# mightypirate1/DRL-Tetris

Measured on AMD Instinct MI355X. Metric: env-steps/sec at 64k parallel 20x10 boards, higher is better.
Workload: dtype u32

## Files before the change

### drl-tetris_amd/csrc/tetris_engine.h

```cpp
#pragma once
#include "tetris_layout.h"
#include "tetris_tables.h"

#if defined(__clang__)
#define TE_UNROLL _Pragma("unroll")
#else
#define TE_UNROLL _Pragma("GCC unroll 8")
#endif

namespace te {

TE_HD int ctz32(uint32_t v) { return __builtin_ctz(v); }
TE_HD int clz32(uint32_t v) { return __builtin_clz(v); }
#if defined(__HIP_DEVICE_COMPILE__)
TE_HD uint32_t ld_stream(const uint32_t* p) { return __builtin_nontemporal_load(p); }
TE_HD void st_stream(uint32_t* p, uint32_t v) { __builtin_nontemporal_store(v, p); }
#else
TE_HD uint32_t ld_stream(const uint32_t* p) { return *p; }
TE_HD void st_stream(uint32_t* p, uint32_t v) { *p = v; }
#endif

#if defined(TE_PATH_COUNTERS) && !defined(__HIPCC__)
enum PathCounter { PC_KICK = 0, PC_KICK_2ND, PC_KICK_3RD, PC_KICK_FAILED, PC_KICK_DOWN, PC_DROP_EXACT, PC_RT_OFF_SPAWN,
                   PC_GARBAGE_ROW, PC_GARBAGE_LIFT2, PC_DEATH_GARBAGE, PC_DEATH_SPAWN, PC_TIMER_LOCK, PC_KEY_KICK, PC_KEY_KICK_FAILED,
                   PC_UNDO_SIMPLE, PC_UNDO_FULL, PC_UNDO_MISPREDICT, PC_NCOUNTERS };
extern unsigned long long te_path_count[PC_NCOUNTERS];
#define TE_COUNT(i) (te_path_count[i]++)
#else
#define TE_COUNT(i) do {} while (0)
#endif

enum MemMode : int { MEM_STREAM = 0, MEM_AGENT = 1, MEM_AFFINE = 2 };
#if defined(__HIP_DEVICE_COMPILE__)
TE_HD uint32_t ld_agent(const uint32_t* p) { return __hip_atomic_load(p, __ATOMIC_RELAXED, __HIP_MEMORY_SCOPE_AGENT); }
TE_HD void st_agent(uint32_t* p, uint32_t v) { __hip_atomic_store(p, v, __ATOMIC_RELAXED, __HIP_MEMORY_SCOPE_AGENT); }
#else
TE_HD uint32_t ld_agent(const uint32_t* p) { return *p; }
TE_HD void st_agent(uint32_t* p, uint32_t v) { *p = v; }
#endif
#if defined(__HIP_DEVICE_COMPILE__)
TE_HD __amdgpu_buffer_rsrc_t te_rsrc(const void* base) {
    return __builtin_amdgcn_make_buffer_rsrc(const_cast<void*>(base), (short)0, -1, 0x00020000);
}
constexpr int TE_AUX_NT = 2, TE_AUX_SC1 = 16;
TE_HD uint32_t ldw_b(const uint32_t* base, uint32_t o, size_t row_bytes, int mem = MEM_STREAM) {
    const __amdgpu_buffer_rsrc_t r = te_rsrc(base);
    if (mem == MEM_AGENT || mem == MEM_AFFINE) return __builtin_amdgcn_raw_buffer_load_b32(r, (int)o, (int)(uint32_t)row_bytes, TE_AUX_SC1);
    return __builtin_amdgcn_raw_buffer_load_b32(r, (int)o, (int)(uint32_t)row_bytes, TE_AUX_NT);
}
TE_HD void stw_b(uint32_t* base, uint32_t o, size_t row_bytes, uint32_t v, int mem = MEM_STREAM) {
    const __amdgpu_buffer_rsrc_t r = te_rsrc(base);
    if (mem == MEM_AGENT) __builtin_amdgcn_raw_buffer_store_b32(v, r, (int)o, (int)(uint32_t)row_bytes, TE_AUX_SC1);
    else if (mem == MEM_AFFINE) __builtin_amdgcn_raw_buffer_store_b32(v, r, (int)o, (int)(uint32_t)row_bytes, 0);
    else __builtin_amdgcn_raw_buffer_store_b32(v, r, (int)o, (int)(uint32_t)row_bytes, TE_AUX_NT);
}
#else
TE_HD uint32_t ldw_b(const uint32_t* base, uint32_t o, size_t row_bytes, int mem = MEM_STREAM) {
    const uint32_t* p = (const uint32_t*)((const char*)base + row_bytes + o);
    return mem != MEM_STREAM ? ld_agent(p) : ld_stream(p);
}
TE_HD void stw_b(uint32_t* base, uint32_t o, size_t row_bytes, uint32_t v, int mem = MEM_STREAM) {
    uint32_t* p = (uint32_t*)((char*)base + row_bytes + o);
    if (mem != MEM_STREAM) st_agent(p, v); else st_stream(p, v);
}
#endif
TE_HD uint32_t ldw(const uint32_t* base, uint32_t o, size_t word_off, int mem = MEM_STREAM) { return ldw_b(base, o, word_off * 4u, mem); }
TE_HD void stw(uint32_t* base, uint32_t o, size_t word_off, uint32_t v, int mem = MEM_STREAM) { stw_b(base, o, word_off * 4u, v, mem); }
struct RowStride { size_t ws; };
template <int N>
struct RowTable { uint32_t bytes[N]; };
TE_HD size_t row_bytes(const RowStride& r, int w) { return (size_t)w * r.ws * 4u; }
template <int N>
TE_HD size_t row_bytes(const RowTable<N>& r, int w) { return r.bytes[w]; }
#if defined(__HIP_DEVICE_COMPILE__)
TE_HD void add_word(uint32_t* p, uint32_t v) { (void)__hip_atomic_fetch_add(p, v, __ATOMIC_RELAXED, __HIP_MEMORY_SCOPE_AGENT); }
#else
TE_HD void add_word(uint32_t* p, uint32_t v) { *p += v; }
#endif
#if defined(__HIP_DEVICE_COMPILE__)
TE_HD uint32_t mul24(uint32_t a, uint32_t b) { return __umul24(a, b); }
#else
TE_HD uint32_t mul24(uint32_t a, uint32_t b) { return a * b; }
#endif
TE_HD int imin(int a, int b) { return a < b ? a : b; }
TE_HD int imax(int a, int b) { return a > b ? a : b; }
TE_HD uint32_t f2u(float f) { union { float f; uint32_t u; } v; v.f = f; return v.u; }
TE_HD float u2f(uint32_t u) { union { float f; uint32_t u; } v; v.u = u; return v.f; }

constexpr uint16_t SHAPE_ROWS[7][4] = {
    {0x2260, 0x0710, 0x3220, 0x4700}, {0x2230, 0x1700, 0x6220, 0x0740}, {0x2640, 0x0630, 0x1320, 0x6300},
    {0x2310, 0x3600, 0x4620, 0x0360}, {0x2222, 0x0f00, 0x4444, 0x00f0}, {0x0720, 0x2320, 0x2700, 0x2620},
    {0x0660, 0x0660, 0x0660, 0x0660},
};
TE_HD int spawn_rot(int kind) { return (int)((0x0977u >> (2 * (kind & 7))) & 3u); }
TE_HD int shape_value(int kind) { return (int)((0x06127534u >> (4 * (kind & 7))) & 15u); }

// ... 71 lines not shown
    int q_loaded;
    Raw8 pf_raw;
    int pf_ok;
};

struct ResetPrefetch { uint32_t seed16; uint64_t word; int ok; };

template <int P>
struct Game {
    Player pl[P];
    uint32_t seed16;
    int round_over, last_winner;
    uint32_t flags;
    uint32_t episode;
    uint32_t steps;
    uint32_t add_lines, add_sent;
    uint32_t status;
    uint32_t draw0, draw1;
};

template <class ROWS>
TE_HD void load_player_rows(const uint32_t* s, uint32_t o, const ROWS& rows, Player& q, bool tint, bool queue = true, int mem = MEM_STREAM,
                            bool errs = true) {
    for (int c = 0; c < NCOL; c++) q.col[c] = ldw_b(s, o, row_bytes(rows, W_COL0 + c), mem);
    if (tint)
        for (int k = 0; k < 3; k++)
            for (int c = 0; c < NCOL; c++) q.tint[k][c] = ldw_b(s, o, row_bytes(rows, W_TINT0 + 10 * k + c), mem);
    uint32_t w = ldw_b(s, o, row_bytes(rows, W_PIECE), mem);
    q.kind = w & 7; q.rot = (w >> 3) & 3; q.x = (int)((w >> 5) & 15) - 4; q.y = (w >> 9) & 31;
    q.next = (w >> 14) & 7; q.dead = (w >> 17) & 1; q.lock_armed = (w >> 18) & 1; q.reward = (w >> 19) & 255;
    w = ldw_b(s, o, row_bytes(rows, W_MISC), mem);
    q.inc_count = w & 255; q.combo_count = (w >> 8) & 255; q.line_count = (w >> 16) & 255;
    q.qlen = (w >> 24) & 15; q.q_overflow = (w >> 28) & 3;
    if (!queue) { q.inc_count = 0; q.qlen = 0; }
    if (!queue && !errs) q.q_overflow = 0;
    q.time_ms = (int32_t)ldw_b(s, o, row_bytes(rows, W_TIME), mem);
    w = ldw_b(s, o, row_bytes(rows, W_DROPCOMBO), mem);
    q.drop_delay = w & 0xFFFF; q.combo_remaining = w >> 16;
    q.drop_time = (int32_t)ldw_b(s, o, row_bytes(rows, W_DROP_TIME), mem);
    q.speedup_time = (int32_t)ldw_b(s, o, row_bytes(rows, W_SPEEDUP_TIME), mem);
    q.lock_time = (int32_t)ldw_b(s, o, row_bytes(rows, W_LOCK_TIME), mem);
    q.combo_start = (int32_t)ldw_b(s, o, row_bytes(rows, W_COMBO_START), mem);
    q.combo_time = (int32_t)ldw_b(s, o, row_bytes(rows, W_COMBO_TIME), mem);
    q.incoming = queue ? u2f(ldw_b(s, o, row_bytes(rows, W_INCOMING), mem)) : 0.0f;
    q.min_remaining = queue ? (int32_t)ldw_b(s, o, row_bytes(rows, W_MIN_REMAINING), mem) : 1000;
    q.piece_draws = ldw_b(s, o, row_bytes(rows, W_PIECE_DRAWS), mem);
    q.hole_draws = queue ? ldw_b(s, o, row_bytes(rows, W_HOLE_DRAWS), mem) : 0u;
    q.pgroup = ldw_b(s, o, row_bytes(rows, W_PIECE_GROUP), mem);
    w = ldw_b(s, o, row_bytes(rows, W_STATS0), mem); q.lines_sent = w & 0xFFFF; q.lines_cleared = w >> 16;
    w = ldw_b(s, o, row_bytes(rows, W_STATS1), mem); q.lines_blocked = w & 0xFFFF; q.max_combo = w >> 16;
    w = ldw_b(s, o, row_bytes(rows, W_STATS2), mem); q.lines_seen = w & 0xFFFF; q.garbage_cleared = w >> 16;
    q.q_loaded = queue && q.qlen > 0;
    q.pf_ok = 0; q.pf_raw.lo = 0; q.pf_raw.hi = 0;
    if (queue)
        for (int i = 0; i < FIFO_CAP; i++) { q.qcount[i] = 0; q.qdelay[i] = 0; }
    if (q.q_loaded) {
        for (int i = 0; i < FIFO_CAP / 2; i++) {
            uint32_t cw = ldw_b(s, o, row_bytes(rows, W_FIFO_COUNT0 + i), mem);
            q.qcount[2 * i] = (int16_t)(cw & 0xFFFF);
            q.qcount[2 * i + 1] = (int16_t)(cw >> 16);
        }
        for (int i = 0; i < FIFO_CAP; i++) q.qdelay[i] = (int32_t)ldw_b(s, o, row_bytes(rows, W_FIFO_DELAY0 + i), mem);
    }
}

TE_HD void load_player(const uint32_t* s, uint32_t o, size_t ws, Player& q, bool tint, bool queue = true, int mem = MEM_STREAM) {
    load_player_rows(s, o, RowStride{ws}, q, tint, queue, mem);
}

template <int P, class ROWS>
TE_HD void load_game_words_rows(const Ref& gr, const ROWS& rows, Game<P>& g, bool counters = false, int mem = MEM_STREAM) {
    uint32_t meta = ldw_b(gr.s, gr.o, row_bytes(rows, G_META), mem);
    g.seed16 = meta & 0xFFFFu;
    g.round_over = (meta >> 16) & 1;
    g.last_winner = (int)((meta >> 17) & 0xF) - 1;
    g.flags = (meta >> 21) & 7u;
    g.episode = ldw_b(gr.s, gr.o, row_bytes(rows, G_EPISODE), mem);
    g.steps = counters ? ldw_b(gr.s, gr.o, row_bytes(rows, G_STEPS), mem) : 0u;
    g.add_lines = 0; g.add_sent = 0;
    g.status = 0;
}

template <int P>
TE_HD void load_game_words(const Ref& gr, Game<P>& g, bool counters = false, int mem = MEM_STREAM) {
    load_game_words_rows<P>(gr, RowStride{gr.ws}, g, counters, mem);
}

template <int P, class ROWS, class GROWS>
TE_HD void load_game_rows(const Geo& geo_in, size_t slot, const ROWS& rows, const GROWS& grows, Game<P>& g, bool tint = false, bool queue = true,
                          bool counters = false, int mem = MEM_STREAM) {
    Geo geo = geo_in;
    geo.P = P;
    load_game_words_rows<P>(game_ref(geo, slot), grows, g, counters, mem);
    TE_UNROLL
    for (int p = 0; p < P; p++) {
        const Ref r = board_ref(geo, p, slot);
        load_player_rows(r.s, r.o, rows, g.pl[p], tint, queue, mem, !counters);
    }
}
template <int P>
TE_HD void load_game(const Geo& geo_in, size_t slot, Game<P>& g, bool tint = false, bool queue = true, bool counters = false, int mem = MEM_STREAM) {
    load_game_rows<P>(geo_in, slot, RowStride{(size_t)P * geo_in.stride}, RowStride{geo_in.stride}, g, tint, queue, counters, mem);
}

template <class ROWS>
TE_HD void store_player_rows(uint32_t* s, uint32_t o, const ROWS& rows, const Player& q, bool tint, bool queue = true, int mem = MEM_STREAM) {
    for (int c = 0; c < NCOL; c++) stw_b(s, o, row_bytes(rows, W_COL0 + c), q.col[c], mem);
    if (tint)
        for (int k = 0; k < 3; k++)
            for (int c = 0; c < NCOL; c++) stw_b(s, o, row_bytes(rows, W_TINT0 + 10 * k + c), q.tint[k][c], mem);
    stw_b(s, o, row_bytes(rows, W_PIECE), (uint32_t)q.kind | ((uint32_t)q.rot << 3) | ((uint32_t)(q.x + 4) << 5) | ((uint32_t)q.y << 9) |
                              ((uint32_t)q.next << 14) | ((uint32_t)q.dead << 17) | ((uint32_t)q.lock_armed << 18) |
                              ((uint32_t)(q.reward & 255) << 19), mem);
    stw_b(s, o, row_bytes(rows, W_MISC), (uint32_t)(q.inc_count & 255) | ((uint32_t)(q.combo_count & 255) << 8) |
                             ((uint32_t)(q.line_count & 255) << 16) | ((uint32_t)q.qlen << 24) | ((uint32_t)q.q_overflow << 28), mem);
    stw_b(s, o, row_bytes(rows, W_TIME), (uint32_t)q.time_ms, mem);
    stw_b(s, o, row_bytes(rows, W_DROPCOMBO), ((uint32_t)q.drop_delay & 0xFFFF) | (q.combo_remaining << 16), mem);
    stw_b(s, o, row_bytes(rows, W_DROP_TIME), (uint32_t)q.drop_time, mem);
    stw_b(s, o, row_bytes(rows, W_SPEEDUP_TIME), (uint32_t)q.speedup_time, mem);
    stw_b(s, o, row_bytes(rows, W_LOCK_TIME), (uint32_t)q.lock_time, mem);
    stw_b(s, o, row_bytes(rows, W_COMBO_START), (uint32_t)q.combo_start, mem);
    stw_b(s, o, row_bytes(rows, W_COMBO_TIME), (uint32_t)q.combo_time, mem);
    if (queue) stw_b(s, o, row_bytes(rows, W_INCOMING), f2u(q.incoming), mem);
    stw_b(s, o, row_bytes(rows, W_MIN_REMAINING), (uint32_t)q.min_remaining, mem);
    stw_b(s, o, row_bytes(rows, W_PIECE_DRAWS), q.piece_draws, mem);
    if (queue) stw_b(s, o, row_bytes(rows, W_HOLE_DRAWS), q.hole_draws, mem);
    stw_b(s, o, row_bytes(rows, W_PIECE_GROUP), q.pgroup, mem);
    stw_b(s, o, row_bytes(rows, W_STATS0), (q.lines_sent & 0xFFFF) | (q.lines_cleared << 16), mem);
    stw_b(s, o, row_bytes(rows, W_STATS1), (q.lines_blocked & 0xFFFF) | (q.max_combo << 16), mem);
    stw_b(s, o, row_bytes(rows, W_STATS2), (q.lines_seen & 0xFFFF) | (q.garbage_cleared << 16), mem);
    if (queue && (q.q_loaded || q.qlen > 0)) {
        for (int i = 0; i < FIFO_CAP / 2; i++)
            stw_b(s, o, row_bytes(rows, W_FIFO_COUNT0 + i), ((uint32_t)q.qcount[2 * i] & 0xFFFF) | ((uint32_t)q.qcount[2 * i + 1] << 16), mem);
        for (int i = 0; i < FIFO_CAP; i++) stw_b(s, o, row_bytes(rows, W_FIFO_DELAY0 + i), (uint32_t)q.qdelay[i], mem);
    }
}

TE_HD void store_player(uint32_t* s, uint32_t o, size_t ws, const Player& q, bool tint, bool queue = true, int mem = MEM_STREAM) {
    store_player_rows(s, o, RowStride{ws}, q, tint, queue, mem);
}

template <int P, class ROWS>
TE_HD void store_game_words_rows(const Ref& gr, const ROWS& rows, const Game<P>& g, bool counters = false, int mem = MEM_STREAM) {
    stw_b(gr.s, gr.o, row_bytes(rows, G_META), g.seed16 | ((uint32_t)g.round_over << 16) | ((uint32_t)(g.last_winner + 1) << 17) | (g.flags << 21), mem);
    stw_b(gr.s, gr.o, row_bytes(rows, G_EPISODE), g.episode, mem);
    if (counters) stw_b(gr.s, gr.o, row_bytes(rows, G_STEPS), g.steps, mem);
    if (g.add_lines) add_word((uint32_t*)((char*)gr.s + row_bytes(rows, G_LINES) + gr.o), g.add_lines);
    if (g.add_sent) add_word((uint32_t*)((char*)gr.s + row_bytes(rows, G_SENT) + gr.o), g.add_sent);
}

template <int P>
TE_HD void store_game_words(const Ref& gr, const Game<P>& g, bool counters = false, int mem = MEM_STREAM) {
    store_game_words_rows<P>(gr, RowStride{gr.ws}, g, counters, mem);
}

template <int P, class ROWS, class GROWS>
TE_HD void store_game_rows(const Geo& geo_in, size_t slot, const ROWS& rows, const GROWS& grows, const Game<P>& g, bool tint = false, bool queue = true,
                           bool counters = false, int mem = MEM_STREAM) {
    Geo geo = geo_in;
    geo.P = P;
    store_game_words_rows<P>(game_ref(geo, slot), grows, g, counters, mem);
    TE_UNROLL
    for (int p = 0; p < P; p++) {
        const Ref r = board_ref(geo, p, slot);
        store_player_rows(r.s, r.o, rows, g.pl[p], tint, queue, mem);
    }
}
template <int P>
TE_HD void store_game(const Geo& geo_in, size_t slot, const Game<P>& g, bool tint = false, bool queue = true, bool counters = false, int mem = MEM_STREAM) {
    store_game_rows<P>(geo_in, slot, RowStride{(size_t)P * geo_in.stride}, RowStride{geo_in.stride}, g, tint, queue, counters, mem);
}


TE_HD uint32_t shape_of(const Ctx& cx, int kind, int rot) { return cx.shapes[(kind << 2) | rot]; }

TE_HD uint64_t band_window(const Ctx& cx, const Player& q, int y) {
    uint32_t lo = 0xFFu, hi = 0xFFFF0000u;
    for (int c = 0; c < 6; c++) lo |= ((uint32_t)((int32_t)(q.col[c] | cx.floor_bits) >> y) & 0xFu) << (4 * c + 8);
    for (int c = 6; c < NCOL; c++) hi |= ((uint32_t)((int32_t)(q.col[c] | cx.floor_bits) >> y) & 0xFu) << (4 * (c - 6));
    return ((uint64_t)hi << 32) | lo;
}

TE_HD bool fits_band(uint64_t band, uint32_t shape, int x) {
    unsigned xs = (unsigned)(x + 2);
// ... 318 lines not shown
    if (q.lock_armed && q.time_ms > q.lock_time && !soft_drop(cx, q)) {
        TE_COUNT(PC_TIMER_LOCK);
        lock_piece(cx, q);
        sent = settle(cx, q, seed16, status);
        finished = true;
    }
    if (!finished) {
        if (cx.queue) {
            int whole = 0;
            while (q.incoming >= 1.0f) { whole++; q.incoming = q.incoming - 1.f; }
            if (whole) q_add(q, whole, q.time_ms, status);
        }
        sent = combo_expire(cx, q, q.time_ms);
        if (sent) {
            if (cx.queue) sent = q_block(q, sent, q.time_ms, false);
            q.lines_sent = (q.lines_sent + (uint32_t)sent) & 0xFFFFu;
        }
        if (cx.queue && q_release(q, q.time_ms))
            if (push_garbage(cx, q, seed16, status)) sent = -1;
    }
    return sent;
}

TE_HD void restart_player(const Ctx& cx, Player& q, uint32_t seed16, uint32_t& status, const ResetPrefetch* pf = nullptr) {
    for (int c = 0; c < NCOL; c++) q.col[c] = 0;
    if (cx.tint)
        for (int k = 0; k < 3; k++)
            for (int c = 0; c < NCOL; c++) q.tint[k][c] = 0;
    q.qlen = 0; q.q_overflow = 0; q.lines_blocked = 0; q.min_remaining = 1000;
    if (cx.queue)
        for (int i = 0; i < FIFO_CAP; i++) { q.qcount[i] = 0; q.qdelay[i] = 0; }
    q.combo_start = 0; q.combo_time = 0; q.max_combo = 0; q.combo_count = 0; q.line_count = 0;
    q.lines_sent = 0; q.lines_cleared = 0; q.garbage_cleared = 0;
    q.speedup_time = 0; q.drop_delay = 1000; q.drop_time = 0; q.lock_time = 0; q.lock_armed = 0;
    q.time_ms = 0; q.incoming = 0.0f; q.lines_seen = 0; q.dead = 0;
    (void)status;
    const uint64_t word = (pf && pf->ok && pf->seed16 == seed16) ? pf->word : cx.start[seed16];
    const uint32_t j = (uint32_t)word & 0xFFu, b0 = ((uint32_t)word >> 8) & 0xFFu, b1 = ((uint32_t)word >> 16) & 0xFFu;
    q.pgroup = (uint32_t)(word >> 32);
    q.kind = (int)(b0 & 7u);
    q.next = (int)(b1 & 7u);
    q.pf_ok = 0;
    q.rot = spawn_rot(q.kind);
    q.x = (NCOL - 4) / 2; q.y = 0;
    q.piece_draws = j + 2; q.hole_draws = 0;
}

template <int P>
TE_HD void reset_game(const Ctx& cx, Game<P>& g, uint32_t seed16, const ResetPrefetch* pf = nullptr) {
    g.round_over = 0;
    int winner = -1, alive = 0;
    TE_UNROLL
    for (int p = 0; p < P; p++)
        if (!g.pl[p].dead) { alive++; winner = p; }
    g.last_winner = winner;
    if (P == 1) g.last_winner = 0;
    if (alive > 1) g.last_winner = -1;
    g.seed16 = seed16 & 0xFFFFu;
    TE_UNROLL
    for (int p = 0; p < P; p++) restart_player(cx, g.pl[p], g.seed16, g.status, pf);
}

TE_HD void prefetch_reset(const Ctx& cx, uint32_t next_seed16, ResetPrefetch& pf) {
    pf.seed16 = next_seed16 & 0xFFFFu;
    pf.word = cx.start[pf.seed16];
    pf.ok = 1;
}

template <int P>
TE_HD void init_game(const Ctx& cx, Game<P>& g, uint32_t seed16) {
    TE_UNROLL
    for (int p = 0; p < P; p++) {
        Player& q = g.pl[p];
        q.reward = 0; q.inc_count = 0; q.combo_remaining = 0; q.dead = 0; q.next = 0; q.kind = 7; q.rot = 0;
        q.q_loaded = 1;
    }
    g.episode = 0; g.steps = 0; g.add_lines = 0; g.add_sent = 0; g.status = 0; g.flags = 0;
    reset_game(cx, g, seed16);
    g.last_winner = -1;
}


TE_HD bool rotate_shape_band(const Ctx& cx, Player& q, int nr, uint32_t shape, uint64_t& b0, uint64_t& b1, bool& b1_ok) {
// ... 530 lines not shown

TE_HD int split_finish(Game<1>& g, int lines_in, bool opp_dead, bool opp_err = false) {
    Player& q = g.pl[0];
    if (g.round_over) return 1;
    if (lines_in > 0) q.incoming = q.incoming + (float)lines_in / 1.0f;
    g.flags = (g.flags & ~SPLIT_OPP_DEAD) | (opp_dead ? SPLIT_OPP_DEAD : 0u);
    int alive = (q.dead ? 0 : 1) + (opp_dead ? 0 : 1);
    if (alive < 2 || q.q_overflow || opp_err) { g.round_over = 1; return 1; }
    return 0;
}

TE_HD void reset_split(const Ctx& cx, Game<1>& g, uint32_t seed16) {
    const int side = (int)(g.flags & SPLIT_SIDE);
    const bool me_alive = !g.pl[0].dead, opp_alive = !(g.flags & SPLIT_OPP_DEAD);
    int winner = -1;
    if (me_alive && !opp_alive) winner = side;
    if (opp_alive && !me_alive) winner = 1 - side;
    reset_game<1>(cx, g, seed16);
    g.last_winner = winner;
    g.flags &= ~SPLIT_OPP_DEAD;
}

TE_HD uint32_t episode_seed(uint32_t game, uint32_t episode) { return (12345u + mul24(7919u, game & 0xFFFFu) + mul24(104729u & 0xFFFFu, episode & 0xFFFFu)) & 0xFFFFu; }

TE_HD void philox4x32_10(uint32_t k0, uint32_t c0, uint32_t c1, uint32_t c2, uint32_t out[4]) {
    uint32_t k1 = 0u, c3 = 0u;
    TE_UNROLL
    for (int r = 0; r < 10; r++) {
        uint64_t p0 = (uint64_t)0xD2511F53u * c0;
        uint64_t p1 = (uint64_t)0xCD9E8D57u * c2;
        uint32_t n0 = (uint32_t)(p1 >> 32) ^ c1 ^ k0;
        uint32_t n1 = (uint32_t)p1;
        uint32_t n2 = (uint32_t)(p0 >> 32) ^ c3 ^ k1;
        uint32_t n3 = (uint32_t)p0;
        c0 = n0; c1 = n1; c2 = n2; c3 = n3;
        k0 += 0x9E3779B9u; k1 += 0xBB67AE85u;
    }
    out[0] = c0; out[1] = c1; out[2] = c2; out[3] = c3;
}

}
```

### drl-tetris_amd/csrc/tetris_hip.hip

```cpp
#include <hip/hip_runtime.h>
#include <hip/hip_ext.h>

#include <math.h>
#include <stdio.h>
#include <stdlib.h>
#include <string.h>

#include <algorithm>
#include <atomic>
#include <mutex>
#include <thread>
#include <new>
#include <chrono>
#include <string>
#include <vector>

#include "tetris_kernels.h"

using namespace te;


#include "tetris_game_kernel.h"

constexpr int CHAIN_LANES = 64;
constexpr int CHAIN_STREAMS = 3;
template <int P, bool AFFINE, bool FUSED>
__device__ __forceinline__ void chain_body(const KArgs& a) {
    __shared__ __attribute__((aligned(16))) uint32_t s_shapes[SHAPE_WORDS];
    const int lane = threadIdx.x;
    if (a.steps < 0) { chain_census(a, lane == 0); return; }
    constexpr int CMEM = AFFINE ? MEM_AFFINE : MEM_AGENT;
    int wave = blockIdx.x;
    uint32_t xcc = 0;
    const auto report_xcc = [&]() { if (AFFINE && blockIdx.x == 0 && lane == 0) st_flag(a.status + F_XCC0 + (a.xcd_slot & 3u), 0x100u | xcc); };
    if (AFFINE) {
        asm volatile("s_getreg_b32 %0, hwreg(HW_REG_XCC_ID)" : "=s"(xcc));
        xcc &= 0xFu;
        if (xcc != ((a.xcd_base + blockIdx.x) & 7u)) {
            if (lane == 0) st_flag(a.status + F_PLACE, 1u);
            report_xcc();
            return;
        }
        wave = (int)((blockIdx.x & ~7u) | xcc);
        if (wave * CHAIN_LANES >= a.n) { report_xcc(); return; }
    }
    const int i = wave * CHAIN_LANES + lane;
    const bool active = lane < CHAIN_LANES && i < a.n;
    LaneCounters cnt = {0, 0, 0, 0};
    const uint32_t shape_word = d_shape_table.s[lane];
    Game<P> g;
    if (active) policy_draw(a, (uint32_t)i, a.first_step, g.draw0, g.draw1);
    const uint32_t d0 = g.draw0, d1 = g.draw1;
    int stride = a.n_stride;
    asm volatile("" : "+s"(stride));
    RowTable<NWORDS> rows = {};
    RowTable<NGWORDS> grows = {};
    if (!FUSED) {
        TE_UNROLL
        for (int w = 0; w < NWORDS; w++)
            if (P > 1 || (w < NWORDS_HOT && w != W_INCOMING && w != W_HOLE_DRAWS)) {
                uint32_t bytes = (uint32_t)(w * P) * (uint32_t)stride * 4u;
                asm volatile("" : "+s"(bytes));
                rows.bytes[w] = bytes;
            }
        TE_UNROLL
        for (int w = 0; w < NGWORDS; w++) {
            uint32_t bytes = (uint32_t)w * (uint32_t)stride * 4u;
            asm volatile("" : "+s"(bytes));
            grows.bytes[w] = bytes;
        }
    }
    const uint32_t seen = chain_poll(a, (uint32_t)wave);
    if (seen == a.epoch - 1u) {
        Geo geo = geo_of(a);
        geo.stride = (size_t)stride;
        if (active) {
            if (FUSED) load_game<P>(geo, (size_t)i, g, false, P > 1, true, CMEM);
            else load_game_rows<P>(geo, (size_t)i, rows, grows, g, false, P > 1, true, CMEM);
            g.draw0 = d0; g.draw1 = d1;
        }
        s_shapes[lane] = shape_word;
        __builtin_amdgcn_wave_barrier();
        if (FUSED) {
            if (active) game_run<P, M_ROLLOUT, false, CMEM>(a, i, s_shapes, g, cnt);
        } else if (active) {
            const Ctx cx = make_ctx(a, s_shapes, false, P > 1);
            rollout_step<P>(cx, a, (size_t)i, a.first_step, g, cnt);
            store_game_rows<P>(geo, (size_t)i, rows, grows, g, false, P > 1, true, CMEM);
            report_status(a, g.status);
        }
        asm volatile("s_waitcnt vmcnt(0)" ::: "memory");
        if (lane == 0) {
            if (AFFINE) st_xcd(a.chain + (size_t)wave * CHAIN_STRIDE, a.epoch);
            else st_agent(a.chain + (size_t)wave * CHAIN_STRIDE, a.epoch);
        }
    } else if (!(seen & CHAIN_ABANDONED)) {
        chain_give_up(a, (uint32_t)wave, lane == 0);
    }
    report_xcc();
}
template <int P>
__global__ __launch_bounds__(64) void k_chain(KArgs a) { chain_body<P, false, false>(a); }
template <int P>
__global__ __launch_bounds__(64) void k_chain_affine(KArgs a) { chain_body<P, true, false>(a); }
template <int P>
__global__ __launch_bounds__(64) void k_chain_fused(KArgs a) { chain_body<P, false, true>(a); }
template <int P>
__global__ __launch_bounds__(64) void k_chain_fused_affine(KArgs a) { chain_body<P, true, true>(a); }
template __global__ void k_chain_affine<1>(KArgs);
template __global__ void k_chain_fused_affine<1>(KArgs);
extern "C" __global__ void tetris_k_xcc_probe(uint32_t* out) {
    if (threadIdx.x == 0) {
        uint32_t xcc;
        asm volatile("s_getreg_b32 %0, hwreg(HW_REG_XCC_ID)" : "=s"(xcc));
        out[blockIdx.x] = xcc & 0xFu;
    }
}
// ... 2845 lines not shown
```

### drl-tetris_amd/csrc/tetris_kernels.h

```cpp
#pragma once
#include "../../include/tetris_hip.h"
#include "tetris_engine.h"

namespace te {

struct KArgs {
    uint32_t* state;
    uint32_t* gstate;
    uint32_t* status;
    const uint8_t* table;
    const uint64_t* start;
    const double* combo_pow;
    uint32_t n_draws, margin;
    int H;
    int n_games;
    int n_stride;
    int n_players;
    int nw;
    int n;
    const int32_t* idx;
    const uint8_t* keys;
    const uint8_t* lens;
    int max_keys;
    const uint8_t* rot;
// ... 58 lines not shown
constexpr uint32_t CHAIN_ABANDONED = 0x80000000u;
constexpr uint32_t CHAIN_EPOCH_MAX = 0x7FFF0000u;
constexpr int CHAIN_STRIDE = 32;
constexpr int CHAIN_SLEEP = 1;
constexpr uint32_t CHAIN_SPIN_LIMIT = 1u << 22;

#if defined(__HIP_DEVICE_COMPILE__)
typedef __attribute__((address_space(1))) uint32_t te_gu32;
TE_HD void or_agent(uint32_t* p, uint32_t v) { (void)__hip_atomic_fetch_or(p, v, __ATOMIC_RELAXED, __HIP_MEMORY_SCOPE_AGENT); }
TE_HD void st_flag(uint32_t* p, uint32_t v) { __hip_atomic_store((te_gu32*)p, v, __ATOMIC_RELAXED, __HIP_MEMORY_SCOPE_SYSTEM); }
TE_HD uint32_t ld_flag(const uint32_t* p) { return __hip_atomic_load((const te_gu32*)p, __ATOMIC_RELAXED, __HIP_MEMORY_SCOPE_SYSTEM); }
TE_HD void st_xcd(uint32_t* p, uint32_t v) { __hip_atomic_store((te_gu32*)p, v, __ATOMIC_RELAXED, __HIP_MEMORY_SCOPE_WAVEFRONT); }
#else
TE_HD void or_agent(uint32_t* p, uint32_t v) { *p |= v; }
TE_HD void st_flag(uint32_t* p, uint32_t v) { *(volatile uint32_t*)p = v; }
TE_HD uint32_t ld_flag(const uint32_t* p) { return *(const volatile uint32_t*)p; }
TE_HD void st_xcd(uint32_t* p, uint32_t v) { *p = v; }
#endif

TE_HD uint32_t chain_poll(const KArgs& a, uint32_t wave) {
    const uint32_t want = a.epoch - 1u;
    const uint32_t* word = a.chain + (size_t)wave * CHAIN_STRIDE;
    uint32_t v = (uint32_t)wave_uniform(ld_agent(word));
    for (uint32_t polls = 1; v != want && !(v & CHAIN_ABANDONED) && polls < a.chain_spin_limit; polls++) {
        if ((polls & 255u) == 0 && wave_uniform(ld_flag(a.status + F_PLACE)) != 0) break;
#if defined(__HIP_DEVICE_COMPILE__)
        __builtin_amdgcn_s_sleep(CHAIN_SLEEP);
#endif
        v = (uint32_t)wave_uniform(ld_agent(word));
    }
    return v;
}
TE_HD void chain_give_up(const KArgs& a, uint32_t wave, bool marker) {
    if (!marker) return;
    or_agent(a.chain + (size_t)wave * CHAIN_STRIDE, CHAIN_ABANDONED);
    st_flag(a.status + F_CHAIN, 1u);
#if defined(__HIP_DEVICE_COMPILE__)
    asm volatile("s_waitcnt vmcnt(0)" ::: "memory");
#endif
}
TE_HD bool chain_wait(const KArgs& a, uint32_t wave, bool marker) {
    const uint32_t seen = chain_poll(a, wave);
    if (seen == a.epoch - 1u) return true;
    if (!(seen & CHAIN_ABANDONED)) chain_give_up(a, wave, marker);
    return false;
}

TE_HD void chain_census(const KArgs& a, bool marker) {
// ... 49 lines not shown
template <int P>
TE_HD void make_rt(const Ctx& cx, Game<P>& g, int player, int r, int t) {
    if (g.round_over) return;
    TE_UNROLL
    for (int p = 0; p < P; p++)
        if (p == player && !g.pl[p].dead) play_rt(cx, g.pl[p], r, t);
}

TE_HD void policy_draw(const KArgs& a, uint32_t slot, unsigned long long step, uint32_t& w0, uint32_t& w1) {
    uint32_t w[4];
    philox4x32_10(a.policy_seed, a.game_offset + slot, (uint32_t)step, (uint32_t)(step >> 32), w);
    w0 = w[0]; w1 = w[1];
}

template <int P, int MODE, bool TINT = false, int MEM = MEM_STREAM>
TE_HD void game_load(const KArgs& a, int i, Game<P>& g) {
    const size_t slot = a.idx ? (size_t)a.idx[i] : (size_t)i;
    if (MODE != M_INIT && MODE != M_SPLIT_INIT)
        load_game<P>(geo_of(a), slot, g, TINT, P > 1 || MODE == M_SPLIT_RESET, MODE == M_ROLLOUT, MEM);
    if (MODE == M_ROLLOUT) policy_draw(a, (uint32_t)slot, a.first_step, g.draw0, g.draw1);
    if (MODE == M_STEP_RT || MODE == M_STEP_RT_AUTO) { g.draw0 = a.rot[i]; g.draw1 = (uint32_t)a.trans[i] | ((a.player ? (uint32_t)a.player[i] : 0u) << 8); }
}

template <int P>
TE_HD void rollout_step(const Ctx& cx, const KArgs& a, size_t slot, unsigned long long step, Game<P>& g, LaneCounters& cnt) {
    TE_UNROLL
    for (int p = 0; p < P; p++) prefetch_next(cx, g.pl[p], g.seed16, g.status);
    ResetPrefetch rpf;
    prefetch_reset(cx, episode_seed(a.game_offset + (uint32_t)slot, g.episode + 1), rpf);
    int r = (int)(g.draw0 & 3u), t = (int)(g.draw1 % 10u);
    int player = P > 1 ? (int)(step % (unsigned long long)P) : 0;
    uint32_t sent_before = 0;
    TE_UNROLL
    for (int p = 0; p < P; p++) sent_before += g.pl[p].lines_sent;
    make_rt<P>(cx, g, player, r, t);
    int done = finish_game<P>(cx, g, a.ms);
    cnt.steps++;
    g.steps++;
    uint32_t sent_after = 0;
    TE_UNROLL
    for (int p = 0; p < P; p++) {
        sent_after += g.pl[p].lines_sent;
        if (!g.pl[p].dead) { cnt.lines += (unsigned)g.pl[p].reward; g.add_lines += (unsigned)g.pl[p].reward; }
    }
    cnt.sent += (sent_after - sent_before) & 0xFFFFu;
    g.add_sent += (sent_after - sent_before) & 0xFFFFu;
    if (done) {
        cnt.episodes++;
        g.episode++;
        reset_game<P>(cx, g, episode_seed(a.game_offset + (uint32_t)slot, g.episode), &rpf);
    }
}

template <int P, int MODE, bool TINT = false, int MEM = MEM_STREAM>
TE_HD void game_run(const KArgs& a, int i, const uint32_t* shapes, Game<P>& g, LaneCounters& cnt) {
    const size_t slot = a.idx ? (size_t)a.idx[i] : (size_t)i;
    Ctx cx = make_ctx(a, shapes, TINT, P > 1 || MODE == M_SPLIT_INIT || MODE == M_SPLIT_RESET);
    if (MODE == M_INIT) init_game<P>(cx, g, (uint32_t)(a.seeds ? (uint16_t)a.seeds[i] : 0));
    if (MODE == M_SPLIT_INIT) {
        init_game<P>(cx, g, (uint32_t)(a.seeds ? (uint16_t)a.seeds[i] : 0));
        g.flags = SPLIT_ON | (a.steps ? SPLIT_SIDE : 0u);
    } else if (MODE == M_SPLIT_RESET) {
        if (P == 1) reset_split(cx, *reinterpret_cast<Game<1>*>(&g), (uint32_t)(a.seeds ? (uint16_t)a.seeds[i] : 0));
    } else if (MODE == M_RESET) {
        reset_game<P>(cx, g, (uint32_t)(a.seeds ? (uint16_t)a.seeds[i] : 0));
    } else if (MODE == M_RESET_SCHED) {
        g.episode++;
        reset_game<P>(cx, g, episode_seed(a.game_offset + (uint32_t)slot, g.episode));
    } else if (MODE == M_MAKE) {
        make_keys<P>(cx, a, i, g);
    } else if (MODE == M_FINISH) {
        TE_UNROLL
        for (int p = 0; p < P; p++) prefetch_next(cx, g.pl[p], g.seed16, g.status);
// ... 442 lines not shown
```

Before: 22.43 billion.

## Hoist buffer descriptors, precompute episode seeds, and defer counter atomics past chain signal

Builds the buffer resource descriptors for the state arrays once per kernel and keeps them in scalar registers, so per-word loads and stores no longer rebuild the descriptor. It also precomputes the game-dependent part of the episode seed and reuses the prefetched reset word unconditionally. Counter atomics and status reporting are moved after the chain epoch signal so they no longer delay the next wave. The chain poll loop is rewritten with a single bounded countdown. The changes cut scalar and vector overhead in a small, latency-bound step, at the cost of more pinned registers and inline asm.

```diff
diff --git a/drl-tetris_amd/csrc/tetris_engine.h b/drl-tetris_amd/csrc/tetris_engine.h
--- a/drl-tetris_amd/csrc/tetris_engine.h
+++ b/drl-tetris_amd/csrc/tetris_engine.h
@@ -39,22 +39,25 @@
 TE_HD void st_agent(uint32_t* p, uint32_t v) { *p = v; }
 #endif
 #if defined(__HIP_DEVICE_COMPILE__)
-TE_HD __amdgpu_buffer_rsrc_t te_rsrc(const void* base) {
+typedef __amdgpu_buffer_rsrc_t te_rsrc_t;
+TE_HD te_rsrc_t te_rsrc(const void* base) {
     return __builtin_amdgcn_make_buffer_rsrc(const_cast<void*>(base), (short)0, -1, 0x00020000);
 }
 constexpr int TE_AUX_NT = 2, TE_AUX_SC1 = 16;
-TE_HD uint32_t ldw_b(const uint32_t* base, uint32_t o, size_t row_bytes, int mem = MEM_STREAM) {
-    const __amdgpu_buffer_rsrc_t r = te_rsrc(base);
+TE_HD uint32_t ldw_rsrc(te_rsrc_t r, uint32_t o, size_t row_bytes, int mem = MEM_STREAM) {
     if (mem == MEM_AGENT || mem == MEM_AFFINE) return __builtin_amdgcn_raw_buffer_load_b32(r, (int)o, (int)(uint32_t)row_bytes, TE_AUX_SC1);
     return __builtin_amdgcn_raw_buffer_load_b32(r, (int)o, (int)(uint32_t)row_bytes, TE_AUX_NT);
 }
-TE_HD void stw_b(uint32_t* base, uint32_t o, size_t row_bytes, uint32_t v, int mem = MEM_STREAM) {
-    const __amdgpu_buffer_rsrc_t r = te_rsrc(base);
+TE_HD void stw_rsrc(te_rsrc_t r, uint32_t o, size_t row_bytes, uint32_t v, int mem = MEM_STREAM) {
     if (mem == MEM_AGENT) __builtin_amdgcn_raw_buffer_store_b32(v, r, (int)o, (int)(uint32_t)row_bytes, TE_AUX_SC1);
     else if (mem == MEM_AFFINE) __builtin_amdgcn_raw_buffer_store_b32(v, r, (int)o, (int)(uint32_t)row_bytes, 0);
     else __builtin_amdgcn_raw_buffer_store_b32(v, r, (int)o, (int)(uint32_t)row_bytes, TE_AUX_NT);
 }
+TE_HD uint32_t ldw_b(const uint32_t* base, uint32_t o, size_t row_bytes, int mem = MEM_STREAM) { return ldw_rsrc(te_rsrc(base), o, row_bytes, mem); }
+TE_HD void stw_b(uint32_t* base, uint32_t o, size_t row_bytes, uint32_t v, int mem = MEM_STREAM) { stw_rsrc(te_rsrc(base), o, row_bytes, v, mem); }
 #else
+struct te_rsrc_t {};
+TE_HD te_rsrc_t te_rsrc(const void*) { return te_rsrc_t{}; }
 TE_HD uint32_t ldw_b(const uint32_t* base, uint32_t o, size_t row_bytes, int mem = MEM_STREAM) {
     const uint32_t* p = (const uint32_t*)((const char*)base + row_bytes + o);
     return mem != MEM_STREAM ? ld_agent(p) : ld_stream(p);
@@ -72,6 +75,20 @@
 TE_HD size_t row_bytes(const RowStride& r, int w) { return (size_t)w * r.ws * 4u; }
 template <int N>
 TE_HD size_t row_bytes(const RowTable<N>& r, int w) { return r.bytes[w]; }
+template <int N>
+struct RowTableR { uint32_t bytes[N]; te_rsrc_t r; };
+template <int N>
+TE_HD size_t row_bytes(const RowTableR<N>& r, int w) { return r.bytes[w]; }
+template <class ROWS>
+TE_HD uint32_t ldw_r(const ROWS& rows, const uint32_t* base, uint32_t o, int w, int mem) { return ldw_b(base, o, row_bytes(rows, w), mem); }
+template <class ROWS>
+TE_HD void stw_r(const ROWS& rows, uint32_t* base, uint32_t o, int w, uint32_t v, int mem) { stw_b(base, o, row_bytes(rows, w), v, mem); }
+#if defined(__HIP_DEVICE_COMPILE__)
+template <int N>
+TE_HD uint32_t ldw_r(const RowTableR<N>& rows, const uint32_t*, uint32_t o, int w, int mem) { return ldw_rsrc(rows.r, o, rows.bytes[w], mem); }
+template <int N>
+TE_HD void stw_r(const RowTableR<N>& rows, uint32_t*, uint32_t o, int w, uint32_t v, int mem) { stw_rsrc(rows.r, o, rows.bytes[w], v, mem); }
+#endif
 #if defined(__HIP_DEVICE_COMPILE__)
 TE_HD void add_word(uint32_t* p, uint32_t v) { (void)__hip_atomic_fetch_add(p, v, __ATOMIC_RELAXED, __HIP_MEMORY_SCOPE_AGENT); }
 #else
@@ -189,45 +206,45 @@
 template <class ROWS>
 TE_HD void load_player_rows(const uint32_t* s, uint32_t o, const ROWS& rows, Player& q, bool tint, bool queue = true, int mem = MEM_STREAM,
                             bool errs = true) {
-    for (int c = 0; c < NCOL; c++) q.col[c] = ldw_b(s, o, row_bytes(rows, W_COL0 + c), mem);
+    for (int c = 0; c < NCOL; c++) q.col[c] = ldw_r(rows, s, o, W_COL0 + c, mem);
     if (tint)
         for (int k = 0; k < 3; k++)
-            for (int c = 0; c < NCOL; c++) q.tint[k][c] = ldw_b(s, o, row_bytes(rows, W_TINT0 + 10 * k + c), mem);
-    uint32_t w = ldw_b(s, o, row_bytes(rows, W_PIECE), mem);
+            for (int c = 0; c < NCOL; c++) q.tint[k][c] = ldw_r(rows, s, o, W_TINT0 + 10 * k + c, mem);
+    uint32_t w = ldw_r(rows, s, o, W_PIECE, mem);
     q.kind = w & 7; q.rot = (w >> 3) & 3; q.x = (int)((w >> 5) & 15) - 4; q.y = (w >> 9) & 31;
     q.next = (w >> 14) & 7; q.dead = (w >> 17) & 1; q.lock_armed = (w >> 18) & 1; q.reward = (w >> 19) & 255;
-    w = ldw_b(s, o, row_bytes(rows, W_MISC), mem);
+    w = ldw_r(rows, s, o, W_MISC, mem);
     q.inc_count = w & 255; q.combo_count = (w >> 8) & 255; q.line_count = (w >> 16) & 255;
     q.qlen = (w >> 24) & 15; q.q_overflow = (w >> 28) & 3;
     if (!queue) { q.inc_count = 0; q.qlen = 0; }
     if (!queue && !errs) q.q_overflow = 0;
-    q.time_ms = (int32_t)ldw_b(s, o, row_bytes(rows, W_TIME), mem);
-    w = ldw_b(s, o, row_bytes(rows, W_DROPCOMBO), mem);
+    q.time_ms = (int32_t)ldw_r(rows, s, o, W_TIME, mem);
+    w = ldw_r(rows, s, o, W_DROPCOMBO, mem);
     q.drop_delay = w & 0xFFFF; q.combo_remaining = w >> 16;
-    q.drop_time = (int32_t)ldw_b(s, o, row_bytes(rows, W_DROP_TIME), mem);
-    q.speedup_time = (int32_t)ldw_b(s, o, row_bytes(rows, W_SPEEDUP_TIME), mem);
-    q.lock_time = (int32_t)ldw_b(s, o, row_bytes(rows, W_LOCK_TIME), mem);
-    q.combo_start = (int32_t)ldw_b(s, o, row_bytes(rows, W_COMBO_START), mem);
-    q.combo_time = (int32_t)ldw_b(s, o, row_bytes(rows, W_COMBO_TIME), mem);
-    q.incoming = queue ? u2f(ldw_b(s, o, row_bytes(rows, W_INCOMING), mem)) : 0.0f;
-    q.min_remaining = queue ? (int32_t)ldw_b(s, o, row_bytes(rows, W_MIN_REMAINING), mem) : 1000;
-    q.piece_draws = ldw_b(s, o, row_bytes(rows, W_PIECE_DRAWS), mem);
-    q.hole_draws = queue ? ldw_b(s, o, row_bytes(rows, W_HOLE_DRAWS), mem) : 0u;
-    q.pgroup = ldw_b(s, o, row_bytes(rows, W_PIECE_GROUP), mem);
-    w = ldw_b(s, o, row_bytes(rows, W_STATS0), mem); q.lines_sent = w & 0xFFFF; q.lines_cleared = w >> 16;
-    w = ldw_b(s, o, row_bytes(rows, W_STATS1), mem); q.lines_blocked = w & 0xFFFF; q.max_combo = w >> 16;
-    w = ldw_b(s, o, row_bytes(rows, W_STATS2), mem); q.lines_seen = w & 0xFFFF; q.garbage_cleared = w >> 16;
+    q.drop_time = (int32_t)ldw_r(rows, s, o, W_DROP_TIME, mem);
+    q.speedup_time = (int32_t)ldw_r(rows, s, o, W_SPEEDUP_TIME, mem);
+    q.lock_time = (int32_t)ldw_r(rows, s, o, W_LOCK_TIME, mem);
+    q.combo_start = (int32_t)ldw_r(rows, s, o, W_COMBO_START, mem);
+    q.combo_time = (int32_t)ldw_r(rows, s, o, W_COMBO_TIME, mem);
+    q.incoming = queue ? u2f(ldw_r(rows, s, o, W_INCOMING, mem)) : 0.0f;
+    q.min_remaining = queue ? (int32_t)ldw_r(rows, s, o, W_MIN_REMAINING, mem) : 1000;
+    q.piece_draws = ldw_r(rows, s, o, W_PIECE_DRAWS, mem);
+    q.hole_draws = queue ? ldw_r(rows, s, o, W_HOLE_DRAWS, mem) : 0u;
+    q.pgroup = ldw_r(rows, s, o, W_PIECE_GROUP, mem);
+    w = ldw_r(rows, s, o, W_STATS0, mem); q.lines_sent = w & 0xFFFF; q.lines_cleared = w >> 16;
+    w = ldw_r(rows, s, o, W_STATS1, mem); q.lines_blocked = w & 0xFFFF; q.max_combo = w >> 16;
+    w = ldw_r(rows, s, o, W_STATS2, mem); q.lines_seen = w & 0xFFFF; q.garbage_cleared = w >> 16;
     q.q_loaded = queue && q.qlen > 0;
     q.pf_ok = 0; q.pf_raw.lo = 0; q.pf_raw.hi = 0;
     if (queue)
         for (int i = 0; i < FIFO_CAP; i++) { q.qcount[i] = 0; q.qdelay[i] = 0; }
     if (q.q_loaded) {
         for (int i = 0; i < FIFO_CAP / 2; i++) {
-            uint32_t cw = ldw_b(s, o, row_bytes(rows, W_FIFO_COUNT0 + i), mem);
+            uint32_t cw = ldw_r(rows, s, o, W_FIFO_COUNT0 + i, mem);
             q.qcount[2 * i] = (int16_t)(cw & 0xFFFF);
             q.qcount[2 * i + 1] = (int16_t)(cw >> 16);
         }
-        for (int i = 0; i < FIFO_CAP; i++) q.qdelay[i] = (int32_t)ldw_b(s, o, row_bytes(rows, W_FIFO_DELAY0 + i), mem);
+        for (int i = 0; i < FIFO_CAP; i++) q.qdelay[i] = (int32_t)ldw_r(rows, s, o, W_FIFO_DELAY0 + i, mem);
     }
 }
 
@@ -237,13 +254,13 @@
 
 template <int P, class ROWS>
 TE_HD void load_game_words_rows(const Ref& gr, const ROWS& rows, Game<P>& g, bool counters = false, int mem = MEM_STREAM) {
-    uint32_t meta = ldw_b(gr.s, gr.o, row_bytes(rows, G_META), mem);
+    uint32_t meta = ldw_r(rows, gr.s, gr.o, G_META, mem);
     g.seed16 = meta & 0xFFFFu;
     g.round_over = (meta >> 16) & 1;
     g.last_winner = (int)((meta >> 17) & 0xF) - 1;
     g.flags = (meta >> 21) & 7u;
-    g.episode = ldw_b(gr.s, gr.o, row_bytes(rows, G_EPISODE), mem);
-    g.steps = counters ? ldw_b(gr.s, gr.o, row_bytes(rows, G_STEPS), mem) : 0u;
+    g.episode = ldw_r(rows, gr.s, gr.o, G_EPISODE, mem);
+    g.steps = counters ? ldw_r(rows, gr.s, gr.o, G_STEPS, mem) : 0u;
     g.add_lines = 0; g.add_sent = 0;
     g.status = 0;
 }
@@ -272,34 +289,34 @@
 
 template <class ROWS>
 TE_HD void store_player_rows(uint32_t* s, uint32_t o, const ROWS& rows, const Player& q, bool tint, bool queue = true, int mem = MEM_STREAM) {
-    for (int c = 0; c < NCOL; c++) stw_b(s, o, row_bytes(rows, W_COL0 + c), q.col[c], mem);
+    for (int c = 0; c < NCOL; c++) stw_r(rows, s, o, W_COL0 + c, q.col[c], mem);
     if (tint)
         for (int k = 0; k < 3; k++)
-            for (int c = 0; c < NCOL; c++) stw_b(s, o, row_bytes(rows, W_TINT0 + 10 * k + c), q.tint[k][c], mem);
-    stw_b(s, o, row_bytes(rows, W_PIECE), (uint32_t)q.kind | ((uint32_t)q.rot << 3) | ((uint32_t)(q.x + 4) << 5) | ((uint32_t)q.y << 9) |
+            for (int c = 0; c < NCOL; c++) stw_r(rows, s, o, W_TINT0 + 10 * k + c, q.tint[k][c], mem);
+    stw_r(rows, s, o, W_PIECE, (uint32_t)q.kind | ((uint32_t)q.rot << 3) | ((uint32_t)(q.x + 4) << 5) | ((uint32_t)q.y << 9) |
                               ((uint32_t)q.next << 14) | ((uint32_t)q.dead << 17) | ((uint32_t)q.lock_armed << 18) |
                               ((uint32_t)(q.reward & 255) << 19), mem);
-    stw_b(s, o, row_bytes(rows, W_MISC), (uint32_t)(q.inc_count & 255) | ((uint32_t)(q.combo_count & 255) << 8) |
+    stw_r(rows, s, o, W_MISC, (uint32_t)(q.inc_count & 255) | ((uint32_t)(q.combo_count & 255) << 8) |
                              ((uint32_t)(q.line_count & 255) << 16) | ((uint32_t)q.qlen << 24) | ((uint32_t)q.q_overflow << 28), mem);
-    stw_b(s, o, row_bytes(rows, W_TIME), (uint32_t)q.time_ms, mem);
-    stw_b(s, o, row_bytes(rows, W_DROPCOMBO), ((uint32_t)q.drop_delay & 0xFFFF) | (q.combo_remaining << 16), mem);
-    stw_b(s, o, row_bytes(rows, W_DROP_TIME), (uint32_t)q.drop_time, mem);
-    stw_b(s, o, row_bytes(rows, W_SPEEDUP_TIME), (uint32_t)q.speedup_time, mem);
-    stw_b(s, o, row_bytes(rows, W_LOCK_TIME), (uint32_t)q.lock_time, mem);
-    stw_b(s, o, row_bytes(rows, W_COMBO_START), (uint32_t)q.combo_start, mem);
-    stw_b(s, o, row_bytes(rows, W_COMBO_TIME), (uint32_t)q.combo_time, mem);
-    if (queue) stw_b(s, o, row_bytes(rows, W_INCOMING), f2u(q.incoming), mem);
-    stw_b(s, o, row_bytes(rows, W_MIN_REMAINING), (uint32_t)q.min_remaining, mem);
-    stw_b(s, o, row_bytes(rows, W_PIECE_DRAWS), q.piece_draws, mem);
-    if (queue) stw_b(s, o, row_bytes(rows, W_HOLE_DRAWS), q.hole_draws, mem);
-    stw_b(s, o, row_bytes(rows, W_PIECE_GROUP), q.pgroup, mem);
-    stw_b(s, o, row_bytes(rows, W_STATS0), (q.lines_sent & 0xFFFF) | (q.lines_cleared << 16), mem);
-    stw_b(s, o, row_bytes(rows, W_STATS1), (q.lines_blocked & 0xFFFF) | (q.max_combo << 16), mem);
-    stw_b(s, o, row_bytes(rows, W_STATS2), (q.lines_seen & 0xFFFF) | (q.garbage_cleared << 16), mem);
+    stw_r(rows, s, o, W_TIME, (uint32_t)q.time_ms, mem);
+    stw_r(rows, s, o, W_DROPCOMBO, ((uint32_t)q.drop_delay & 0xFFFF) | (q.combo_remaining << 16), mem);
+    stw_r(rows, s, o, W_DROP_TIME, (uint32_t)q.drop_time, mem);
+    stw_r(rows, s, o, W_SPEEDUP_TIME, (uint32_t)q.speedup_time, mem);
+    stw_r(rows, s, o, W_LOCK_TIME, (uint32_t)q.lock_time, mem);
+    stw_r(rows, s, o, W_COMBO_START, (uint32_t)q.combo_start, mem);
+    stw_r(rows, s, o, W_COMBO_TIME, (uint32_t)q.combo_time, mem);
+    if (queue) stw_r(rows, s, o, W_INCOMING, f2u(q.incoming), mem);
+    stw_r(rows, s, o, W_MIN_REMAINING, (uint32_t)q.min_remaining, mem);
+    stw_r(rows, s, o, W_PIECE_DRAWS, q.piece_draws, mem);
+    if (queue) stw_r(rows, s, o, W_HOLE_DRAWS, q.hole_draws, mem);
+    stw_r(rows, s, o, W_PIECE_GROUP, q.pgroup, mem);
+    stw_r(rows, s, o, W_STATS0, (q.lines_sent & 0xFFFF) | (q.lines_cleared << 16), mem);
+    stw_r(rows, s, o, W_STATS1, (q.lines_blocked & 0xFFFF) | (q.max_combo << 16), mem);
+    stw_r(rows, s, o, W_STATS2, (q.lines_seen & 0xFFFF) | (q.garbage_cleared << 16), mem);
     if (queue && (q.q_loaded || q.qlen > 0)) {
         for (int i = 0; i < FIFO_CAP / 2; i++)
-            stw_b(s, o, row_bytes(rows, W_FIFO_COUNT0 + i), ((uint32_t)q.qcount[2 * i] & 0xFFFF) | ((uint32_t)q.qcount[2 * i + 1] << 16), mem);
-        for (int i = 0; i < FIFO_CAP; i++) stw_b(s, o, row_bytes(rows, W_FIFO_DELAY0 + i), (uint32_t)q.qdelay[i], mem);
+            stw_r(rows, s, o, W_FIFO_COUNT0 + i, ((uint32_t)q.qcount[2 * i] & 0xFFFF) | ((uint32_t)q.qcount[2 * i + 1] << 16), mem);
+        for (int i = 0; i < FIFO_CAP; i++) stw_r(rows, s, o, W_FIFO_DELAY0 + i, (uint32_t)q.qdelay[i], mem);
     }
 }
 
@@ -307,13 +324,18 @@
     store_player_rows(s, o, RowStride{ws}, q, tint, queue, mem);
 }
 
+template <class ROWS>
+TE_HD void add_game_counters(const Ref& gr, const ROWS& rows, uint32_t add_lines, uint32_t add_sent) {
+    if (add_lines) add_word((uint32_t*)((char*)gr.s + row_bytes(rows, G_LINES) + gr.o), add_lines);
+    if (add_sent) add_word((uint32_t*)((char*)gr.s + row_bytes(rows, G_SENT) + gr.o), add_sent);
+}
+
 template <int P, class ROWS>
-TE_HD void store_game_words_rows(const Ref& gr, const ROWS& rows, const Game<P>& g, bool counters = false, int mem = MEM_STREAM) {
-    stw_b(gr.s, gr.o, row_bytes(rows, G_META), g.seed16 | ((uint32_t)g.round_over << 16) | ((uint32_t)(g.last_winner + 1) << 17) | (g.flags << 21), mem);
-    stw_b(gr.s, gr.o, row_bytes(rows, G_EPISODE), g.episode, mem);
-    if (counters) stw_b(gr.s, gr.o, row_bytes(rows, G_STEPS), g.steps, mem);
-    if (g.add_lines) add_word((uint32_t*)((char*)gr.s + row_bytes(rows, G_LINES) + gr.o), g.add_lines);
-    if (g.add_sent) add_word((uint32_t*)((char*)gr.s + row_bytes(rows, G_SENT) + gr.o), g.add_sent);
+TE_HD void store_game_words_rows(const Ref& gr, const ROWS& rows, const Game<P>& g, bool counters = false, int mem = MEM_STREAM, bool adds = true) {
+    stw_r(rows, gr.s, gr.o, G_META, g.seed16 | ((uint32_t)g.round_over << 16) | ((uint32_t)(g.last_winner + 1) << 17) | (g.flags << 21), mem);
+    stw_r(rows, gr.s, gr.o, G_EPISODE, g.episode, mem);
+    if (counters) stw_r(rows, gr.s, gr.o, G_STEPS, g.steps, mem);
+    if (adds) add_game_counters(gr, rows, g.add_lines, g.add_sent);
 }
 
 template <int P>
@@ -323,10 +345,10 @@
 
 template <int P, class ROWS, class GROWS>
 TE_HD void store_game_rows(const Geo& geo_in, size_t slot, const ROWS& rows, const GROWS& grows, const Game<P>& g, bool tint = false, bool queue = true,
-                           bool counters = false, int mem = MEM_STREAM) {
+                           bool counters = false, int mem = MEM_STREAM, bool adds = true) {
     Geo geo = geo_in;
     geo.P = P;
-    store_game_words_rows<P>(game_ref(geo, slot), grows, g, counters, mem);
+    store_game_words_rows<P>(game_ref(geo, slot), grows, g, counters, mem, adds);
     TE_UNROLL
     for (int p = 0; p < P; p++) {
         const Ref r = board_ref(geo, p, slot);
@@ -691,7 +713,7 @@
     return sent;
 }
 
-TE_HD void restart_player(const Ctx& cx, Player& q, uint32_t seed16, uint32_t& status, const ResetPrefetch* pf = nullptr) {
+TE_HD void restart_player(const Ctx& cx, Player& q, uint32_t seed16, uint32_t& status, const ResetPrefetch* pf = nullptr, bool pf_sure = false) {
     for (int c = 0; c < NCOL; c++) q.col[c] = 0;
     if (cx.tint)
         for (int k = 0; k < 3; k++)
@@ -704,7 +726,7 @@
     q.speedup_time = 0; q.drop_delay = 1000; q.drop_time = 0; q.lock_time = 0; q.lock_armed = 0;
     q.time_ms = 0; q.incoming = 0.0f; q.lines_seen = 0; q.dead = 0;
     (void)status;
-    const uint64_t word = (pf && pf->ok && pf->seed16 == seed16) ? pf->word : cx.start[seed16];
+    const uint64_t word = (pf && (pf_sure || (pf->ok && pf->seed16 == seed16))) ? pf->word : cx.start[seed16];
     const uint32_t j = (uint32_t)word & 0xFFu, b0 = ((uint32_t)word >> 8) & 0xFFu, b1 = ((uint32_t)word >> 16) & 0xFFu;
     q.pgroup = (uint32_t)(word >> 32);
     q.kind = (int)(b0 & 7u);
@@ -716,7 +738,7 @@
 }
 
 template <int P>
-TE_HD void reset_game(const Ctx& cx, Game<P>& g, uint32_t seed16, const ResetPrefetch* pf = nullptr) {
+TE_HD void reset_game(const Ctx& cx, Game<P>& g, uint32_t seed16, const ResetPrefetch* pf = nullptr, bool pf_sure = false) {
     g.round_over = 0;
     int winner = -1, alive = 0;
     TE_UNROLL
@@ -727,7 +749,7 @@
     if (alive > 1) g.last_winner = -1;
     g.seed16 = seed16 & 0xFFFFu;
     TE_UNROLL
-    for (int p = 0; p < P; p++) restart_player(cx, g.pl[p], g.seed16, g.status, pf);
+    for (int p = 0; p < P; p++) restart_player(cx, g.pl[p], g.seed16, g.status, pf, pf_sure);
 }
 
 TE_HD void prefetch_reset(const Ctx& cx, uint32_t next_seed16, ResetPrefetch& pf) {
@@ -1304,6 +1326,17 @@
 }
 
 TE_HD uint32_t episode_seed(uint32_t game, uint32_t episode) { return (12345u + mul24(7919u, game & 0xFFFFu) + mul24(104729u & 0xFFFFu, episode & 0xFFFFu)) & 0xFFFFu; }
+TE_HD uint32_t episode_seed_game(uint32_t game) { return 12345u + mul24(7919u, game & 0xFFFFu); }
+TE_HD uint32_t episode_seed_of(uint32_t game_half, uint32_t episode) {
+#if defined(__HIP_DEVICE_COMPILE__)
+    uint32_t e;
+    asm("v_mul_u32_u24 %0, 0x9919, %1" : "=v"(e) : "v"(episode & 0xFFFFu));
+    static_assert((104729u & 0xFFFFu) == 0x9919u, "episode_seed");
+    return (game_half + e) & 0xFFFFu;
+#else
+    return (game_half + mul24(104729u & 0xFFFFu, episode & 0xFFFFu)) & 0xFFFFu;
+#endif
+}
 
 TE_HD void philox4x32_10(uint32_t k0, uint32_t c0, uint32_t c1, uint32_t c2, uint32_t out[4]) {
     uint32_t k1 = 0u, c3 = 0u;
diff --git a/drl-tetris_amd/csrc/tetris_hip.hip b/drl-tetris_amd/csrc/tetris_hip.hip
--- a/drl-tetris_amd/csrc/tetris_hip.hip
+++ b/drl-tetris_amd/csrc/tetris_hip.hip
@@ -24,6 +24,12 @@
 
 constexpr int CHAIN_LANES = 64;
 constexpr int CHAIN_STREAMS = 3;
+template <class T>
+__device__ __forceinline__ const T* pin_global(const T* p) {
+    unsigned long long u = (unsigned long long)p;
+    asm volatile("" : "+s"(u));
+    return (const T*)(const __attribute__((address_space(1))) T*)u;
+}
 template <int P, bool AFFINE, bool FUSED>
 __device__ __forceinline__ void chain_body(const KArgs& a) {
     __shared__ __attribute__((aligned(16))) uint32_t s_shapes[SHAPE_WORDS];
@@ -53,9 +59,15 @@
     const uint32_t d0 = g.draw0, d1 = g.draw1;
     int stride = a.n_stride;
     asm volatile("" : "+s"(stride));
-    RowTable<NWORDS> rows = {};
-    RowTable<NGWORDS> grows = {};
+    static_assert(FUSED || P == 1, "one board per game: its rows start at KArgs::state");
+    RowTableR<NWORDS> rows = {};
+    RowTableR<NGWORDS> grows = {};
     if (!FUSED) {
+        rows.r = te_rsrc(a.state);
+        grows.r = te_rsrc(a.gstate);
+#if defined(__HIP_DEVICE_COMPILE__)
+        asm volatile("" : "+s"(rows.r), "+s"(grows.r));
+#endif
         TE_UNROLL
         for (int w = 0; w < NWORDS; w++)
             if (P > 1 || (w < NWORDS_HOT && w != W_INCOMING && w != W_HOLE_DRAWS)) {
@@ -70,6 +82,15 @@
             grows.bytes[w] = bytes;
         }
     }
+    StepAhead ahead = {0, a.ms};
+    Ctx cx = make_ctx(a, s_shapes, false, P > 1);
+    if (!FUSED) {
+        ahead.seed_game = episode_seed_game(a.game_offset + (uint32_t)i);
+        asm volatile("" : "+v"(ahead.seed_game));
+        asm volatile("" : "+s"(ahead.ms));
+        asm volatile("" : "+s"(cx.floor_bits));
+        cx.table = pin_global(cx.table); cx.start = pin_global(cx.start); cx.combo_pow = pin_global(cx.combo_pow);
+    }
     const uint32_t seen = chain_poll(a, (uint32_t)wave);
     if (seen == a.epoch - 1u) {
         Geo geo = geo_of(a);
@@ -84,15 +105,20 @@
         if (FUSED) {
             if (active) game_run<P, M_ROLLOUT, false, CMEM>(a, i, s_shapes, g, cnt);
         } else if (active) {
-            const Ctx cx = make_ctx(a, s_shapes, false, P > 1);
-            rollout_step<P>(cx, a, (size_t)i, a.first_step, g, cnt);
-            store_game_rows<P>(geo, (size_t)i, rows, grows, g, false, P > 1, true, CMEM);
-            report_status(a, g.status);
+            rollout_step<P>(cx, a, (size_t)i, a.first_step, g, cnt, &ahead);
+            store_game_rows<P>(geo, (size_t)i, rows, grows, g, false, P > 1, true, CMEM, false);
         }
         asm volatile("s_waitcnt vmcnt(0)" ::: "memory");
         if (lane == 0) {
             if (AFFINE) st_xcd(a.chain + (size_t)wave * CHAIN_STRIDE, a.epoch);
             else st_agent(a.chain + (size_t)wave * CHAIN_STRIDE, a.epoch);
+        }
+        if (!FUSED && active) {
+            add_game_counters(game_ref(geo, (size_t)i), grows, g.add_lines, g.add_sent);
+            if (g.status) {
+                report_status(a, g.status);
+                asm volatile("s_waitcnt vmcnt(0)" ::: "memory");
+            }
         }
     } else if (!(seen & CHAIN_ABANDONED)) {
         chain_give_up(a, (uint32_t)wave, lane == 0);
diff --git a/drl-tetris_amd/csrc/tetris_kernels.h b/drl-tetris_amd/csrc/tetris_kernels.h
--- a/drl-tetris_amd/csrc/tetris_kernels.h
+++ b/drl-tetris_amd/csrc/tetris_kernels.h
@@ -104,8 +104,12 @@
     const uint32_t want = a.epoch - 1u;
     const uint32_t* word = a.chain + (size_t)wave * CHAIN_STRIDE;
     uint32_t v = (uint32_t)wave_uniform(ld_agent(word));
-    for (uint32_t polls = 1; v != want && !(v & CHAIN_ABANDONED) && polls < a.chain_spin_limit; polls++) {
-        if ((polls & 255u) == 0 && wave_uniform(ld_flag(a.status + F_PLACE)) != 0) break;
+    if (v == want) return v;
+    const uint32_t bound = a.chain_spin_limit - 1u;
+    int32_t left = (int32_t)(bound < 0x7FFFFFFFu ? bound : 0x7FFFFFFFu);
+    while (imin((int32_t)(v ^ want), left) > 0) {
+        if ((left & 255) == 0 && wave_uniform(ld_flag(a.status + F_PLACE)) != 0) left = 1;
+        left--;
 #if defined(__HIP_DEVICE_COMPILE__)
         __builtin_amdgcn_s_sleep(CHAIN_SLEEP);
 #endif
@@ -201,19 +205,22 @@
     if (MODE == M_STEP_RT || MODE == M_STEP_RT_AUTO) { g.draw0 = a.rot[i]; g.draw1 = (uint32_t)a.trans[i] | ((a.player ? (uint32_t)a.player[i] : 0u) << 8); }
 }
 
+struct StepAhead { uint32_t seed_game; int ms; };
 template <int P>
-TE_HD void rollout_step(const Ctx& cx, const KArgs& a, size_t slot, unsigned long long step, Game<P>& g, LaneCounters& cnt) {
+TE_HD void rollout_step(const Ctx& cx, const KArgs& a, size_t slot, unsigned long long step, Game<P>& g, LaneCounters& cnt,
+                        const StepAhead* ahead = nullptr) {
     TE_UNROLL
     for (int p = 0; p < P; p++) prefetch_next(cx, g.pl[p], g.seed16, g.status);
+    const uint32_t next_seed = episode_seed_of(ahead ? ahead->seed_game : episode_seed_game(a.game_offset + (uint32_t)slot), g.episode + 1);
     ResetPrefetch rpf;
-    prefetch_reset(cx, episode_seed(a.game_offset + (uint32_t)slot, g.episode + 1), rpf);
+    prefetch_reset(cx, next_seed, rpf);
     int r = (int)(g.draw0 & 3u), t = (int)(g.draw1 % 10u);
     int player = P > 1 ? (int)(step % (unsigned long long)P) : 0;
     uint32_t sent_before = 0;
     TE_UNROLL
     for (int p = 0; p < P; p++) sent_before += g.pl[p].lines_sent;
     make_rt<P>(cx, g, player, r, t);
-    int done = finish_game<P>(cx, g, a.ms);
+    int done = finish_game<P>(cx, g, ahead ? ahead->ms : a.ms);
     cnt.steps++;
     g.steps++;
     uint32_t sent_after = 0;
@@ -227,7 +234,7 @@
     if (done) {
         cnt.episodes++;
         g.episode++;
-        reset_game<P>(cx, g, episode_seed(a.game_offset + (uint32_t)slot, g.episode), &rpf);
+        reset_game<P>(cx, g, next_seed, &rpf, true);
     }
 }
 
```

New measurement: 23.29 billion (median of 6 runs). 1.04x the previous value.
